# txthpc/amg

Measured on AMD Instinct MI355X. Metric: V-cycle iters/sec + fine-level SpMV GB/s (%HBM peak), 64M-row 7pt Poisson, higher is better.
Workload: dtype f64

## Files before the change

### amg_amd/_native.py

```python
from __future__ import annotations

import ctypes as C
import os
from pathlib import Path

import numpy as np

ROOT = Path(__file__).resolve().parent.parent
LIB_PATH = Path(os.environ["SSS_AMG_LIB"]) if os.environ.get("SSS_AMG_LIB") else ROOT / "amg_amd" / "lib" / "libsss_amg.so"
BIN_PATH = ROOT / "amg_amd" / "bin" / "amg"

_dbl_p = C.POINTER(C.c_double)
_int_p = C.POINTER(C.c_int)


class SSS_MAT(C.Structure):
    _fields_ = [("num_rows", C.c_int), ("num_cols", C.c_int), ("num_nnzs", C.c_int),
                ("row_ptr", _int_p), ("col_idx", _int_p), ("val", _dbl_p)]


class SSS_IMAT(C.Structure):
    _fields_ = [("num_rows", C.c_int), ("num_cols", C.c_int), ("num_nnzs", C.c_int),
                ("row_ptr", _int_p), ("col_idx", _int_p), ("val", _int_p)]


class SSS_VEC(C.Structure):
    _fields_ = [("n", C.c_int), ("d", _dbl_p)]


class SSS_IVEC(C.Structure):
    _fields_ = [("n", C.c_int), ("d", _int_p)]


class SSS_RTN(C.Structure):
    _fields_ = [("ares", C.c_double), ("rres", C.c_double), ("nits", C.c_int)]


class SSS_AMG_PARS(C.Structure):
    _fields_ = [("cycle_type", C.c_int), ("tol", C.c_double), ("ctol", C.c_double), ("max_it", C.c_int),
                ("cs_type", C.c_int), ("max_levels", C.c_int), ("coarse_dof", C.c_int), ("smoother", C.c_int),
                ("relax", C.c_double), ("cf_order", C.c_int), ("pre_iter", C.c_int), ("post_iter", C.c_int),
                ("poly_deg", C.c_int), ("interp_type", C.c_int), ("strong_threshold", C.c_double),
                ("max_row_sum", C.c_double), ("trunc_threshold", C.c_double)]


class SSS_AMG_COMP(C.Structure):
    _fields_ = [("A", SSS_MAT), ("R", SSS_MAT), ("P", SSS_MAT), ("b", SSS_VEC), ("x", SSS_VEC),
                ("cfmark", SSS_IVEC), ("wp", SSS_VEC)]


class SSS_AMG(C.Structure):
    _fields_ = [("num_levels", C.c_int), ("cg", C.POINTER(SSS_AMG_COMP)), ("pars", SSS_AMG_PARS),
                ("rtn", SSS_RTN)]


class SSS_SMTR(C.Structure):
    _fields_ = [("smoother", C.c_int), ("A", C.POINTER(SSS_MAT)), ("b", C.POINTER(SSS_VEC)),
                ("x", C.POINTER(SSS_VEC)), ("relax", C.c_double), ("nsweeps", C.c_int), ("istart", C.c_int),
                ("iend", C.c_int), ("istep", C.c_int), ("ndeg", C.c_int), ("cf_order", C.c_int),
                ("ordering", _int_p)]


class SSS_KRYLOV(C.Structure):
    _fields_ = [("tol", C.c_double), ("A", C.POINTER(SSS_MAT)), ("b", C.POINTER(SSS_VEC)),
                ("u", C.POINTER(SSS_VEC)), ("restart", C.c_int), ("matrix", C.c_int), ("stop_type", C.c_int)]


class SSS_HIP_OPTS(C.Structure):
    _fields_ = [("device", C.c_int), ("smoother", C.c_int), ("coarse", C.c_int), ("row_cap", C.c_int),
                ("use_graph", C.c_int), ("verbose", C.c_int),
                ("inner", C.c_int), ("inner_from", C.c_int), ("relabel", C.c_int),
                ("sorted_tiles", C.c_int), ("sum_order", C.c_int), ("inner_long", C.c_int), ("formats", C.c_int)]

FORMATS = {"auto": -1, "full": 0, "lean": 1}


class SSS_HIP_LEVEL_INFO(C.Structure):
    _fields_ = [("rows", C.c_int), ("nnz", C.c_int), ("nnz_p", C.c_int), ("dag_f", C.c_int),
                ("dag_c", C.c_int), ("smoother_kind", C.c_int), ("gs_engine_f", C.c_int), ("gs_engine_c", C.c_int),
                ("gs_stall", C.c_int), ("a_format", C.c_int), ("a_stream_bytes", C.c_longlong),
                ("inner", C.c_int), ("r_format", C.c_int), ("p_format", C.c_int), ("pad_", C.c_int)]


SMOOTH = {"exact": 0, "hybrid": 1, "jacobi": 2}
COARSE_RS, COARSE_PMIS = 1, 3
COARSE = {"krylov": 0, "direct": 1}
VEC = {"b": 0, "x": 1, "wp": 2}
SPMV = {"mxy": 0, "amxpy": 1, "resid": 2, "acc": 3}

ABI_SYMBOLS = [
    "SSS_amg_solve", "SSS_amg_cycle", "SSS_amg_coarest_solve", "SSS_amg_smoother_pre", "SSS_amg_smoother_post",
    "SSS_blas_mv_amxpy", "SSS_blas_mv_mxy", "SSS_solver_amg", "SSS_get_time", "SSS_free", "SSS_blas_vec_norm2",
    "SSS_print_itinfo", "SSS_exit_on_errcode", "SSS_blas_array_norm2", "SSS_blas_array_dot", "SSS_blas_array_axpy",
    "SSS_blas_array_norminf", "SSS_blas_array_set", "SSS_blas_array_axpby", "SSS_blas_array_ax", "SSS_vec_create",
    "SSS_vec_set_value", "SSS_mat_destroy", "SSS_vec_destroy", "SSS_calloc", "SSS_amg_data_create",
    "SSS_ivec_create", "SSS_mat_struct_create", "SSS_vec_cp", "SSS_iarray_cp", "SSS_blas_array_cp", "SSS_mat_cp",
    "SSS_mat_get_diag", "SSS_ivec_destroy", "SSS_amg_data_destroy", "SSS_imat_trans", "SSS_iarray_set",
    "SSS_imat_destroy", "SSS_mat_trans", "SSS_blas_mat_rap", "SSS_realloc", "SSS_amg_complexity_print",
    "SSS_amg_setup", "SSS_amg_coarsen", "SSS_amg_interp", "SSS_amg_interp_trunc", "interp_DIR", "SSS_mat_read",
    "SSS_amg_pars_init", "SSS_amg_pars_print", "mmio_info", "mmio_data",
    "sss_hip_opts_default", "sss_hip_device_count", "sss_hip_mem_info", "sss_hip_hier_create", "sss_hip_hier_destroy",
    "sss_hip_setup_create", "sss_amg_setup_hooked", "sss_hip_rap", "sss_hip_pmis", "sss_pmis_host",
    "sss_hip_std_pattern", "sss_std_pattern_host", "sss_hip_interp_std",
    "sss_hip_upload_vec", "sss_hip_download_vec", "sss_hip_cycle", "sss_hip_residual_norm", "sss_hip_pcg",
    "sss_hip_fgmres", "sss_hip_host_orth",
    "SSS_amg_save", "SSS_amg_load",
    "sss_hip_coarse_solve", "sss_hip_smooth", "sss_hip_sync", "sss_hip_level_info_get", "sss_hip_num_levels", "sss_hip_tail_from",
    "sss_hip_cycle_launches", "sss_hip_cycle_bytes",
    "sss_hip_spmv_plan_create", "sss_hip_spmv_plan_destroy", "sss_hip_spmv", "sss_hip_host_spmv",
    "sss_hip_host_smooth", "sss_hip_host_coarse_solve", "sss_hip_host_cache_clear", "sss_hip_time_level0_spmv", "sss_hip_time_iterations",
    "sss_hip_time_level0_spmv_csr", "sss_hip_time_levels", "sss_hip_dist_time_tail_levels",
    "sss_gen_stencil",
    "sss_hip_rccl_unique_id", "sss_hip_comm_rccl", "sss_hip_comm_host", "sss_hip_comm_timing", "sss_hip_comm_destroy",
    "sss_hip_dist_create", "sss_hip_dist_destroy", "sss_hip_dist_info", "sss_hip_dist_level_flags",
    "sss_hip_dist_upload_vec",
    "sss_hip_dist_download_vec", "sss_hip_dist_cycle", "sss_hip_dist_residual_norm", "sss_hip_dist_sync",
    "sss_hip_dist_time_level0_spmv", "sss_hip_dist_time_levels", "sss_hip_dist_halo_stats",
    "sss_part_plan_create", "sss_part_plan_destroy", "sss_part_save", "sss_part_plan_load",
    "sss_hip_dist_create_from_files", "sss_hip_dist_level_size", "sss_part_plan_nagg", "sss_part_plan_level",
    "sss_part_plan_matrix", "sss_part_plan_ids", "sss_part_plan_halo",
]

_ip, _dp = C.POINTER(C.c_int), C.POINTER(C.c_double)
EXCHANGE_FN = C.CFUNCTYPE(C.c_int, C.c_void_p, C.c_int, _ip, _ip, _dp, C.c_int, _ip, _ip, _dp)
ALLREDUCE_FN = C.CFUNCTYPE(C.c_int, C.c_void_p, _dp, C.c_int)
ALLGATHERV_FN = C.CFUNCTYPE(C.c_int, C.c_void_p, _dp, C.c_int, _dp, _ip, _ip)


A_FORMATS = {0: "CSR (12 B/entry)", 1: "column-sorted tiles (12 B/entry)", 2: "dictionary tiles (4 B/entry)",
             3: "value-dictionary sorted tiles (5 B/entry)"}


def a_format_name(code: int) -> str:
    if code & 64:
        return "dictionary ELL (1 B/entry, padded rows)"
    if code & 128:
        return "column ELL (4 B/entry, padded rows)"
    return A_FORMATS.get(code & 3, A_FORMATS[0])


class SSS_HIP_HOST_TRANSPORT(C.Structure):
    _fields_ = [("ctx", C.c_void_p), ("exchange", EXCHANGE_FN), ("allreduce_sum", ALLREDUCE_FN),
                ("allgatherv", ALLGATHERV_FN)]

_lib = None


def _declare(lib):
    P = C.POINTER
    sig = {
        "SSS_amg_pars_init": (None, [P(SSS_AMG_PARS)]),
        "SSS_amg_pars_print": (None, [P(SSS_AMG_PARS)]),
        "SSS_amg_setup": (None, [P(SSS_AMG), P(SSS_MAT), P(SSS_AMG_PARS)]),
        "SSS_amg_data_destroy": (None, [P(SSS_AMG)]),
        "SSS_amg_solve": (SSS_RTN, [P(SSS_AMG), P(SSS_VEC), P(SSS_VEC)]),
        "SSS_print_itinfo": (None, [C.c_int, C.c_int, C.c_double, C.c_double, C.c_double]),
        "SSS_amg_cycle": (None, [P(SSS_AMG)]),
        "SSS_solver_amg": (SSS_RTN, [P(SSS_MAT), P(SSS_VEC), P(SSS_VEC), P(SSS_AMG_PARS)]),
        "SSS_mat_read": (None, [C.c_char_p, P(SSS_MAT)]),
        "SSS_mat_destroy": (None, [P(SSS_MAT)]),
        "SSS_mat_trans": (SSS_MAT, [P(SSS_MAT)]),
        "SSS_blas_mat_rap": (SSS_MAT, [P(SSS_MAT), P(SSS_MAT), P(SSS_MAT)]),
        "SSS_amg_coarsen": (C.c_int, [P(SSS_MAT), P(SSS_IVEC), P(SSS_MAT), P(SSS_IMAT), P(SSS_AMG_PARS)]),
        "SSS_amg_interp": (None, [P(SSS_MAT), P(SSS_IVEC), P(SSS_MAT), P(SSS_IMAT), P(SSS_AMG_PARS)]),
        "SSS_ivec_create": (SSS_IVEC, [C.c_int]),
        "SSS_blas_mv_amxpy": (None, [C.c_double, P(SSS_MAT), P(SSS_VEC), P(SSS_VEC)]),
        "SSS_blas_mv_mxy": (None, [P(SSS_MAT), P(SSS_VEC), P(SSS_VEC)]),
        "mmio_info": (C.c_int, [_int_p, _int_p, _int_p, _int_p, C.c_char_p]),
        "mmio_data": (C.c_int, [_int_p, _int_p, _dbl_p, C.c_char_p]),
        "sss_gen_stencil": (C.c_int, [C.c_int] * 6 + [P(SSS_MAT)]),
        "sss_hip_opts_default": (None, [P(SSS_HIP_OPTS)]),
        "sss_hip_device_count": (C.c_int, []),
        "sss_hip_mem_info": (C.c_int, [P(C.c_size_t), P(C.c_size_t)]),
        "sss_hip_hier_create": (C.c_void_p, [P(SSS_AMG), P(SSS_HIP_OPTS)]),
        "sss_hip_setup_create": (C.c_void_p, [P(SSS_AMG), P(SSS_MAT), P(SSS_AMG_PARS), P(SSS_HIP_OPTS),
                                              P(C.c_double)]),
        "sss_hip_hier_destroy": (None, [C.c_void_p]),
        "sss_hip_rap": (C.c_int, [P(SSS_MAT), P(SSS_MAT), P(SSS_MAT), P(SSS_MAT)]),
        "sss_hip_pmis": (C.c_int, [P(SSS_IMAT), _int_p, _int_p, _int_p]),
        "sss_pmis_host": (C.c_int, [P(SSS_IMAT), _int_p, _int_p, _int_p]),
        "sss_hip_std_pattern": (C.c_int, [P(SSS_IMAT), _int_p, C.c_int, P(SSS_MAT)]),
        "sss_std_pattern_host": (C.c_int, [P(SSS_IMAT), _int_p, C.c_int, P(SSS_MAT)]),
        "sss_hip_interp_std": (C.c_int, [P(SSS_MAT), P(SSS_IMAT), _int_p, P(SSS_MAT), C.c_double]),
        "SSS_mat_struct_create": (SSS_MAT, [C.c_int, C.c_int, C.c_int]),
        "sss_hip_upload_vec": (C.c_int, [C.c_void_p, C.c_int, C.c_int, _dbl_p, C.c_int]),
        "sss_hip_download_vec": (C.c_int, [C.c_void_p, C.c_int, C.c_int, _dbl_p, C.c_int]),
        "sss_hip_cycle": (C.c_int, [C.c_void_p]),
        "sss_hip_residual_norm": (C.c_int, [C.c_void_p, _dbl_p]),
        "sss_hip_pcg": (C.c_int, [C.c_void_p, C.c_double, C.c_int, P(C.c_int), _dbl_p, _dbl_p, C.c_int]),
        "sss_hip_fgmres": (C.c_int, [C.c_void_p, C.c_double, C.c_int, C.c_int, P(C.c_int), _dbl_p, _dbl_p, C.c_int]),
        "sss_hip_host_orth": (C.c_int, [C.c_int, C.c_int, _dbl_p, _dbl_p, _dbl_p, _dbl_p]),
        "SSS_amg_save": (C.c_int, [P(SSS_AMG), C.c_char_p]),
        "SSS_amg_load": (C.c_int, [P(SSS_AMG), C.c_char_p]),
        "sss_hip_coarse_solve": (C.c_int, [C.c_void_p]),
        "sss_hip_smooth": (C.c_int, [C.c_void_p, C.c_int, C.c_int]),
        "sss_hip_sync": (C.c_int, [C.c_void_p]),
        "sss_hip_level_info_get": (C.c_int, [C.c_void_p, C.c_int, P(SSS_HIP_LEVEL_INFO)]),
        "sss_hip_num_levels": (C.c_int, [C.c_void_p]),
        "sss_hip_tail_from": (C.c_int, [C.c_void_p]),
        "sss_hip_cycle_launches": (C.c_int, [C.c_void_p]),
        "sss_hip_cycle_bytes": (C.c_int, [C.c_void_p, C.POINTER(C.c_double), C.c_int]),
        "sss_hip_host_spmv": (C.c_int, [C.c_int, C.c_double, P(SSS_MAT), _dbl_p, _dbl_p, _dbl_p, C.c_int]),
        "sss_hip_host_smooth": (C.c_int, [P(SSS_SMTR), C.c_int]),
        "sss_hip_host_coarse_solve": (C.c_int, [P(SSS_MAT), P(SSS_VEC), P(SSS_VEC), C.c_double, C.c_int,
                                                C.c_int]),
        "sss_hip_time_level0_spmv": (C.c_int, [C.c_void_p, C.c_int, _dbl_p]),
        "sss_hip_time_level0_spmv_csr": (C.c_int, [C.c_void_p, C.c_int, _dbl_p]),
        "sss_hip_time_levels": (C.c_int, [C.c_void_p, C.c_int, _dbl_p, C.c_int]),
        "sss_hip_dist_time_tail_levels": (C.c_int, [C.c_void_p, C.c_int, _dbl_p, C.c_int]),
        "sss_hip_time_iterations": (C.c_int, [C.c_void_p, C.c_int, _dbl_p, _dbl_p]),
        "sss_hip_rccl_unique_id": (C.c_int, [C.c_char_p]),
        "sss_hip_comm_rccl": (C.c_void_p, [C.c_int, C.c_int, C.c_char_p, C.c_int]),
        "sss_hip_comm_host": (C.c_void_p, [C.c_int, C.c_int, P(SSS_HIP_HOST_TRANSPORT)]),
        "sss_hip_comm_timing": (C.c_void_p, [C.c_int, C.c_int]),
        "sss_hip_comm_destroy": (None, [C.c_void_p]),
        "sss_hip_dist_create": (C.c_void_p, [P(SSS_AMG), P(SSS_HIP_OPTS), C.c_void_p, C.c_int]),
        "sss_hip_dist_destroy": (None, [C.c_void_p]),
        "sss_hip_dist_info": (C.c_int, [C.c_void_p, _int_p, _int_p, _int_p, _int_p]),
        "sss_hip_dist_level_size": (C.c_int, [C.c_void_p, C.c_int, _int_p, _int_p, P(C.c_longlong)]),
        "sss_hip_dist_level_flags": (C.c_int, [C.c_void_p, C.c_int]),
        "sss_hip_dist_upload_vec": (C.c_int, [C.c_void_p, C.c_int, _dbl_p, C.c_int]),
        "sss_hip_dist_download_vec": (C.c_int, [C.c_void_p, C.c_int, _dbl_p, C.c_int]),
        "sss_hip_dist_cycle": (C.c_int, [C.c_void_p]),
        "sss_hip_dist_residual_norm": (C.c_int, [C.c_void_p, _dbl_p]),
        "sss_hip_dist_sync": (C.c_int, [C.c_void_p]),
        "sss_hip_dist_time_level0_spmv": (C.c_int, [C.c_void_p, C.c_int, _dbl_p]),
        "sss_hip_dist_time_levels": (C.c_int, [C.c_void_p, C.c_int, _dbl_p, _dbl_p, C.c_int]),
        "sss_hip_dist_halo_stats": (C.c_int, [C.c_void_p, P(C.c_longlong), P(C.c_longlong), C.c_int, C.c_int,
                                              _int_p, _int_p, _int_p]),
        "sss_part_plan_create": (C.c_void_p, [P(SSS_AMG), C.c_int, C.c_int, C.c_int]),
        "sss_part_save": (C.c_int, [P(SSS_AMG), C.c_int, C.c_int, C.c_char_p]),
        "sss_part_plan_load": (C.c_void_p, [C.c_char_p]),
        "sss_hip_dist_create_from_files": (C.c_void_p, [C.c_char_p, P(SSS_HIP_OPTS), C.c_void_p]),
        "sss_part_plan_destroy": (None, [C.c_void_p]),
        "sss_part_plan_nagg": (C.c_int, [C.c_void_p]),
        "sss_part_plan_level": (C.c_int, [C.c_void_p, C.c_int, _int_p, _int_p, _int_p, _int_p]),
        "sss_part_plan_matrix": (C.c_int, [C.c_void_p, C.c_int, C.c_int, P(SSS_MAT)]),
        "sss_part_plan_ids": (C.c_int, [C.c_void_p, C.c_int, P(_int_p), P(_int_p)]),
        "sss_part_plan_halo": (C.c_int, [C.c_void_p, C.c_int, _int_p, P(_int_p), P(_int_p), P(_int_p), _int_p,
                                         P(_int_p), P(_int_p)]),
    }
    for name, (res, args) in sig.items():
        fn = getattr(lib, name)
        fn.restype = res
        fn.argtypes = args
    return lib


def lib():
    global _lib
    if _lib is None:
        if not LIB_PATH.exists():
            raise RuntimeError(f"{LIB_PATH} is missing: run `make` (or __graft_entry__.build())")
        _lib = _declare(C.CDLL(str(LIB_PATH)))
    return _lib


def dptr(a: np.ndarray):
    assert a.dtype == np.float64 and a.flags["C_CONTIGUOUS"]
    return a.ctypes.data_as(_dbl_p)


def iptr(a: np.ndarray):
    assert a.dtype == np.int32 and a.flags["C_CONTIGUOUS"]
    return a.ctypes.data_as(_int_p)


def csr_arrays(M: SSS_MAT, copy: bool = True):
    n, nnz = M.num_rows, M.num_nnzs
    rp = np.ctypeslib.as_array(M.row_ptr, shape=(n + 1,))
    ci = np.ctypeslib.as_array(M.col_idx, shape=(nnz,)) if nnz else np.zeros(0, np.int32)
    v = np.ctypeslib.as_array(M.val, shape=(nnz,)) if nnz else np.zeros(0, np.float64)
    return (rp.copy(), ci.copy(), v.copy()) if copy else (rp, ci, v)


class NumpyCSR:

    def __init__(self, rp, ci, v, ncols=None):
        self.rp = np.ascontiguousarray(rp, dtype=np.int32)
        self.ci = np.ascontiguousarray(ci, dtype=np.int32)
        self.v = np.ascontiguousarray(v, dtype=np.float64)
        n = len(self.rp) - 1
        self.mat = SSS_MAT(n, n if ncols is None else ncols, len(self.v), iptr(self.rp), iptr(self.ci),
                           dptr(self.v))


def default_pars() -> SSS_AMG_PARS:
    p = SSS_AMG_PARS()
    lib().SSS_amg_pars_init(C.byref(p))
    return p


def pmis(rp, ci, device: bool = False):
    rp = np.ascontiguousarray(rp, dtype=np.int32)
    ci = np.ascontiguousarray(ci, dtype=np.int32)
    n = len(rp) - 1
    S = SSS_IMAT(n, n, len(ci), iptr(rp), iptr(ci) if len(ci) else None, None)
    mark = np.full(max(n, 1), -7, np.int32)
    nc, rounds = C.c_int(-1), C.c_int(-1)
    fn = lib().sss_hip_pmis if device else lib().sss_pmis_host
    rc = fn(C.byref(S), iptr(mark), C.byref(nc), C.byref(rounds))
    if rc != 0:
        err = RuntimeError(f"PMIS split failed ({rc})")
        err.rc, err.mark = rc, mark[:n]
        raise err
    return mark[:n], nc.value, rounds.value


def _imat(rp, ci):
    rp = np.ascontiguousarray(rp, dtype=np.int32)
    ci = np.ascontiguousarray(ci, dtype=np.int32)
    n = len(rp) - 1
    return SSS_IMAT(n, n, len(ci), iptr(rp), iptr(ci) if len(ci) else None, None), (rp, ci)


def std_pattern(rp, ci, mark, device: bool = False):
    S, keep = _imat(rp, ci)
    mark = np.ascontiguousarray(mark, dtype=np.int32)
    P = SSS_MAT()
    fn = lib().sss_hip_std_pattern if device else lib().sss_std_pattern_host
    rc = fn(C.byref(S), iptr(mark), int((mark == 1).sum()), C.byref(P))
    if rc != 0:
        err = RuntimeError(f"standard pattern failed ({rc})")
        err.rc = rc
        raise err
    prp, pci, _ = csr_arrays(P)
    lib().SSS_mat_destroy(C.byref(P))
    return prp, pci


def interp_std(A_csr, S_csr, mark, P_pattern, trunc: float, device: bool = False):
    Am = NumpyCSR(*A_csr)
    S, keep = _imat(*S_csr)
    mark = np.ascontiguousarray(mark, dtype=np.int32)
    prp = np.ascontiguousarray(P_pattern[0], dtype=np.int32)
    pci = np.ascontiguousarray(P_pattern[1], dtype=np.int32)
    n = len(prp) - 1
    P = lib().SSS_mat_struct_create(n, int((mark == 1).sum()), len(pci))
    C.memmove(P.row_ptr, prp.ctypes.data, prp.nbytes)
    if len(pci):
        C.memmove(P.col_idx, pci.ctypes.data, pci.nbytes)
    try:
        if device:
            rc = lib().sss_hip_interp_std(C.byref(Am.mat), C.byref(S), iptr(mark), C.byref(P), trunc)
            if rc != 0:
                err = RuntimeError(f"standard interpolation failed ({rc})")
                err.rc = rc
                raise err
        else:
            pars = default_pars()
            pars.interp_type, pars.trunc_threshold = 2, trunc
            verts = SSS_IVEC(len(mark), iptr(mark))
            lib().SSS_amg_interp(C.byref(Am.mat), C.byref(verts), C.byref(P), C.byref(S), C.byref(pars))
        return (*csr_arrays(P), P.num_cols)
    finally:
        lib().SSS_mat_destroy(C.byref(P))


def generate(kind: int, n: int, nz: int | None = None, z0: int = 0, z1: int | None = None) -> SSS_MAT:
    nz = n if nz is None else nz
    z1 = nz if z1 is None else z1
    A = SSS_MAT()
    rc = lib().sss_gen_stencil(kind, n, n, nz, z0, z1, C.byref(A))
    if rc != 0:
        raise RuntimeError(f"sss_gen_stencil failed ({rc})")
    return A


def read_mtx(path: str | os.PathLike) -> SSS_MAT:
    A = SSS_MAT()
    lib().SSS_mat_read(str(path).encode(), C.byref(A))
    return A


class Hierarchy:

    def __init__(self, A: SSS_MAT | None, pars: SSS_AMG_PARS | None = None):
        self.pars = pars if pars is not None else default_pars()
        self.mg = SSS_AMG()
        if A is not None:
            lib().SSS_amg_setup(C.byref(self.mg), C.byref(A), C.byref(self.pars))

    def save(self, path) -> None:
        rc = lib().SSS_amg_save(C.byref(self.mg), str(path).encode())
        if rc != 0:
            raise OSError(f"SSS_amg_save({path}) failed ({rc})")

    @classmethod
    def load(cls, path) -> "Hierarchy":
        H = cls(None)
        rc = lib().SSS_amg_load(C.byref(H.mg), str(path).encode())
        if rc != 0:
            raise OSError(f"SSS_amg_load({path}) failed ({rc})")
        H.pars = H.mg.pars
        return H

# ... 425 lines not shown
```

### amg_amd/csrc/sss_hier.hip

```cpp
#include "sss_engine.hpp"
#include "sss_tail.hpp"

#include <atomic>
#include <condition_variable>
#include <mutex>
#include <thread>

#include <chrono>

#include <cmath>

#include <algorithm>
#include <cstdlib>
#include <cstring>
#include <string>
#include <thread>
#include <vector>

using namespace sss;

struct sss_hip_hier {
    int nl = 0;
    SSS_AMG_PARS pars{};
    sss_hip_opts opts{};
// ... 1420 lines not shown
    SSS_HIP(hipEventElapsedTime(&ms, h->ev0, h->ev1));
    *avg_ms = (double)ms / reps;
    return 0;
}

extern "C" int sss_hip_time_iterations(sss_hip_hier *h, int reps, double *avg_ms, double *absres)
{
    SSS_HIP(hipStreamSynchronize(h->stream));
    SSS_HIP(hipEventRecord(h->ev0, h->stream));
    for (int r = 0; r < reps; ++r) {
        int rc = sss_hip_cycle(h);
        if (!rc) rc = sss_hip_residual_norm(h, absres);
        if (rc) return rc;
    }
    SSS_HIP(hipEventRecord(h->ev1, h->stream));
    SSS_HIP(hipEventSynchronize(h->ev1));
    float ms = 0.f;
    SSS_HIP(hipEventElapsedTime(&ms, h->ev0, h->ev1));
    *avg_ms = (double)ms / reps;
    return 0;
}

extern char **environ;

namespace {
struct HostCSR {
    DevCSR d;
    ~HostCSR() { devcsr_free(d); }
};
struct HostSmooth {
    std::mutex run;
    DevCSR d;
    SmootherPlan sp;
    ~HostSmooth()
    {
        smoother_free(sp);
        devcsr_free(d);
    }
};
struct HostCoarse {
    std::mutex run;
    DevCSR d;
    CoarseDirect cd;
    bool direct = false;
    CoarseKrylov *k = nullptr;
    ~HostCoarse()
    {
        if (direct) coarse_direct_free(cd);
        coarse_krylov_destroy(k);
        devcsr_free(d);
    }
};

inline unsigned long long mix64(unsigned long long h, unsigned long long w)
{
    h ^= w * 0x9E3779B97F4A7C15ull;
    h = (h << 31) | (h >> 33);
    return h * 0xC2B2AE3D27D4EB4Full;
}
unsigned long long hash_bytes(const void *p, size_t n, unsigned long long seed)
{
    const unsigned char *b = static_cast<const unsigned char *>(p);
    constexpr size_t kChunk = (size_t)1 << 20;
    const int nc = (int)((n + kChunk - 1) / kChunk);
    std::vector<unsigned long long> part((size_t)std::max(nc, 1), 0);
    parallel_chunks(nc, 1, [&](int c0, int c1) {
        for (int c = c0; c < c1; ++c) {
            const size_t lo = (size_t)c * kChunk, hi = std::min(n, lo + kChunk);
            unsigned long long h = 0x2545F4914F6CDD1Dull ^ (unsigned long long)c;
            size_t i = lo;
            for (; i + 8 <= hi; i += 8) {
                unsigned long long w;
                std::memcpy(&w, b + i, 8);
                h = mix64(h, w);
            }
            for (; i < hi; ++i) h = mix64(h, b[i]);
            part[(size_t)c] = h;
        }
    });
    unsigned long long h = mix64(seed, n);
    for (auto v : part) h = mix64(h, v);
    return h;
}
unsigned long long matrix_key(const SSS_MAT &A, unsigned long long use)
{
    int dev = 0;
    (void)hipGetDevice(&dev);
    unsigned long long h = mix64(mix64(use, (unsigned long long)dev), (unsigned long long)A.num_rows);
    for (char **e = environ; e && *e; ++e)
        if (std::strncmp(*e, "SSS_HIP_", 8) == 0) h = hash_bytes(*e, std::strlen(*e), h);
    h = mix64(h, (unsigned long long)A.num_cols);
    h = mix64(h, (unsigned long long)A.num_nnzs);
    h = hash_bytes(A.row_ptr, sizeof(int) * ((size_t)A.num_rows + 1), h);
    h = hash_bytes(A.col_idx, sizeof(int) * (size_t)A.num_nnzs, h);
    return hash_bytes(A.val, sizeof(double) * (size_t)A.num_nnzs, h);
}

struct PreparedCache {
    struct Entry {
        unsigned long long key;
        std::shared_ptr<void> obj;
        unsigned long long tick;
    };
    std::mutex mu;
    std::vector<Entry> e;
    unsigned long long tick = 0;
    static constexpr size_t kMax = 4;
    template <class T, class Build>
    std::shared_ptr<T> get(unsigned long long key, Build build, bool cache = true)
    {
        if (!cache) return build();
        {
            std::lock_guard<std::mutex> lk(mu);
            for (auto &x : e)
                if (x.key == key) {
                    x.tick = ++tick;
                    return std::static_pointer_cast<T>(x.obj);
                }
        }
        std::shared_ptr<T> obj = build();
        if (!obj) return obj;
        std::lock_guard<std::mutex> lk(mu);
        if (e.size() >= kMax) {
            auto old = std::min_element(e.begin(), e.end(), [](const Entry &a, const Entry &b) { return a.tick < b.tick; });
            e.erase(old);
        }
        e.push_back({key, obj, ++tick});
        return obj;
    }
    void clear()
    {
        std::lock_guard<std::mutex> lk(mu);
        e.clear();
    }
};
bool cacheable(const SSS_MAT &A)
{
    const char *e = getenv("SSS_HIP_HOST_CACHE_MB");
    const double mb = (e && *e) ? atof(e) : 1024.0;
    return 12.0 * (double)A.num_nnzs + 4.0 * (double)A.num_rows <= mb * 1048576.0;
}
PreparedCache &prepared()
{
    static PreparedCache *c = new PreparedCache();
    return *c;
}
}

extern "C" void sss_hip_host_cache_clear(void) { prepared().clear(); }

extern "C" int sss_hip_host_spmv(int op, double alpha, const SSS_MAT *A, const double *x, const double *b,
                                 double *y, int cap)
{
    if (sss_hip_device_count() <= 0) return ERROR_MISC;
    sss_hip_opts o;
    sss_hip_opts_default(&o);
    int enc = level_encoding(o) & (kEncSortedTiles | kEncDict);
    if (A->num_rows != A->num_cols) enc = restriction_encoding(o) & (kEncSortedTiles | kEncEll);
    auto M = prepared().get<HostCSR>(matrix_key(*A, 0x5350ull ^ ((unsigned long long)enc << 8)), [&] {
        auto m = std::make_shared<HostCSR>();
        return devcsr_upload(m->d, *A, -1, enc) ? nullptr : m;
    }, cacheable(*A));
    if (!M) return ERROR_MISC;
    const size_t ny = (size_t)A->num_rows, nx = (size_t)A->num_cols;
    double *dx = dev_alloc<double>(nx), *dy = dev_alloc<double>(ny), *db = dev_alloc<double>(ny);
    int rc = 0;
    if (!dx || !dy || !db) rc = ERROR_ALLOC_MEM;
    if (!rc && hipMemcpy(dx, x, sizeof(double) * nx, hipMemcpyHostToDevice) != hipSuccess) rc = ERROR_MISC;
    if (!rc && hipMemcpy(dy, y, sizeof(double) * ny, hipMemcpyHostToDevice) != hipSuccess) rc = ERROR_MISC;
    if (!rc && b && hipMemcpy(db, b, sizeof(double) * ny, hipMemcpyHostToDevice) != hipSuccess) rc = ERROR_MISC;
    if (!rc) rc = launch_spmv(M->d, op, alpha, dx, db, dy, cap, nullptr, nullptr);
    if (!rc && hipMemcpy(y, dy, sizeof(double) * ny, hipMemcpyDeviceToHost) != hipSuccess) rc = ERROR_MISC;
    dev_free(dx);
    dev_free(dy);
    dev_free(db);
    return rc;
}

extern "C" int sss_hip_host_smooth(const SSS_SMTR *s, int post)
{
    if (sss_hip_device_count() <= 0) return ERROR_MISC;
    const int n = s->A->num_rows;
    const int use_cf = s->cf_order && s->ordering;
    const bool natural = !use_cf && s->smoother == SSS_SM_GS;
    const int i1 = post ? s->iend : s->istart, in = post ? s->istart : s->iend, step = s->istep;
    if (natural && step != 1 && step != -1) {
        fprintf(stderr, "### ERROR: natural-order Gauss-Seidel on the GPU needs istep = +1 or -1 (got %d)\n", step);
        return ERROR_INPUT_PAR;
    }
    const bool desc = step < 0;
    const int lo = desc ? in : i1, hi = (desc ? i1 : in) + 1;
    if (natural && (lo < 0 || hi > n)) return ERROR_INPUT_PAR;
    if (natural && lo >= hi) return 0;
    const int kind = s->smoother == SSS_SM_JACOBI ? SSS_HIP_SMOOTH_JACOBI : SSS_HIP_SMOOTH_EXACT;
    unsigned long long use = mix64(0x534Dull, natural ? 1 : 0);
    use = mix64(use, (unsigned long long)kind);
    if (natural) use = mix64(mix64(use, (unsigned long long)lo), (unsigned long long)hi);
    if (use_cf) use = hash_bytes(s->ordering, sizeof(int) * (size_t)n, use);
    auto M = prepared().get<HostSmooth>(matrix_key(*s->A, use), [&] {
        auto m = std::make_shared<HostSmooth>();
        if (devcsr_upload(m->d, *s->A)) return std::shared_ptr<HostSmooth>();
        if (natural ? smoother_build_natural(m->sp, *s->A, lo, hi)
                    : smoother_build(m->sp, *s->A, use_cf ? s->ordering : nullptr, kind))
            return std::shared_ptr<HostSmooth>();
        return m;
    }, cacheable(*s->A));
    if (!M) return ERROR_MISC;
    std::lock_guard<std::mutex> run_lock(M->run);
    double *dx = dev_alloc<double>((size_t)n), *db = dev_alloc<double>((size_t)n);
    int rc = (!dx || !db) ? ERROR_ALLOC_MEM : 0;
    if (!rc && hipMemcpy(dx, s->x->d, sizeof(double) * n, hipMemcpyHostToDevice) != hipSuccess) rc = ERROR_MISC;
    if (!rc && hipMemcpy(db, s->b->d, sizeof(double) * n, hipMemcpyHostToDevice) != hipSuccess) rc = ERROR_MISC;
    bool x_zero = !natural;
    for (int i = 0; x_zero && i < n; ++i) {
        unsigned long long u;
        memcpy(&u, s->x->d + i, sizeof u);
        x_zero = u == 0ull;
    }
    if (!rc) rc = smoother_run(M->sp, M->d, db, dx, s->nsweeps, nullptr, nullptr, nullptr, nullptr, x_zero, natural && desc);
    if (!rc && hipMemcpy(s->x->d, dx, sizeof(double) * n, hipMemcpyDeviceToHost) != hipSuccess) rc = ERROR_MISC;
    bool stalled = false;
    for (auto &ps : M->sp.pass) {
        unsigned e = 0;
        if (gs_persist_error(ps, &e)) rc = rc ? rc : ERROR_MISC;
        if (e) {
            (void)hipMemset(ps.gp.err, 0, sizeof(unsigned));
            stalled = true;
        }
    }
    unsigned ez = 0;
    if (gs_fused_error(M->sp.fz, &ez, true)) rc = rc ? rc : ERROR_MISC;
    if (ez) stalled = true;
    if (stalled && !rc) rc = stall_error("SSS_amg_smoother_pre/post");
    dev_free(dx);
    dev_free(db);
    return rc;
}

extern "C" int sss_hip_host_coarse_solve(SSS_MAT *A, SSS_VEC *b, SSS_VEC *x, double ctol, int coarse_mode,
                                         int row_cap)
{
    if (sss_hip_device_count() <= 0) return ERROR_MISC;
    const int n = A->num_rows;
    const bool direct = coarse_mode == SSS_HIP_COARSE_DIRECT && n <= 20000;
    auto M = prepared().get<HostCoarse>(
        matrix_key(*A, mix64(mix64(0x4353ull, direct ? 1 : 0), (unsigned long long)row_cap)), [&] {
            auto m = std::make_shared<HostCoarse>();
            if (devcsr_upload(m->d, *A)) return std::shared_ptr<HostCoarse>();
            if (direct) {
                if (coarse_direct_build(m->cd, *A, nullptr)) return std::shared_ptr<HostCoarse>();
                m->direct = true;
            } else {
                m->k = coarse_krylov_create(m->d, row_cap, nullptr);
                if (!m->k) return std::shared_ptr<HostCoarse>();
            }
            return m;
        }, cacheable(*A));
    if (!M) return ERROR_MISC;
    std::lock_guard<std::mutex> run_lock(M->run);
    double *dx = dev_alloc<double>((size_t)n), *db = dev_alloc<double>((size_t)n);
    int rc = (!dx || !db) ? ERROR_ALLOC_MEM : 0;
    if (!rc && hipMemcpy(dx, x->d, sizeof(double) * n, hipMemcpyHostToDevice) != hipSuccess) rc = ERROR_MISC;
    if (!rc && hipMemcpy(db, b->d, sizeof(double) * n, hipMemcpyHostToDevice) != hipSuccess) rc = ERROR_MISC;
    if (!rc) {
        if (direct) {
            rc = coarse_direct_apply(M->cd, db, dx, nullptr);
            if (!rc && hipDeviceSynchronize() != hipSuccess) rc = ERROR_MISC;
        } else {
            rc = coarse_krylov_solve(M->k, M->d, db, dx, ctol, nullptr);
        }
    }
    if (!rc && hipMemcpy(x->d, dx, sizeof(double) * n, hipMemcpyDeviceToHost) != hipSuccess) rc = ERROR_MISC;
    dev_free(dx);
    dev_free(db);
    return rc;
}
```

### amg_amd/csrc/sss_spmv_dev.hpp

```cpp
#pragma once

#include "sss_engine.hpp"

namespace sss {

__device__ __forceinline__ int xcd_bid() { return blockIdx.x; }

struct SpmvSmem {
    alignas(16) double v[kTileEntries];
    double red[kBlock / 64];
    double d[kBlock];
};

struct DictSmem {
    int dd[256];
    double vd[256];
    unsigned char rowof[kTileEntries];
};
struct DevDict {
    const unsigned *code = nullptr;
    const int4 *pd = nullptr;
    const int *dd = nullptr;
    const double *vd = nullptr;
    const unsigned *pk = nullptr;
// ... 680 lines not shown
        const double acc = long_row_chunks(
            k0, k1, b[i], [=, &sm](int base, int m) { stage_products(sm.v, base, base + m, ci, v, x); },
            [&sm](int, int m, double acc) { return threadIdx.x == 0 ? chain_sub(acc, sm.v, 0, m) : acc; });
        if (threadIdx.x == 0) epi(r0, i, acc);
    }
}
constexpr int kWaveStage = 256;
constexpr int kWaveRowMin = 600;
constexpr int kFreeRowMin = 300;

__device__ __forceinline__ void wave_sync()
{
    __builtin_amdgcn_fence(__ATOMIC_RELEASE, "wavefront");
    __builtin_amdgcn_wave_barrier();
    __builtin_amdgcn_fence(__ATOMIC_ACQUIRE, "wavefront");
}

template <bool SUB, class Prod>
__device__ __forceinline__ double wave_row_chain(int k0, int k1, const int *__restrict__ ci,
                                                 const double *__restrict__ v, Prod prod, double init,
                                                 double *strip)
{
    constexpr int U = kWaveStage / 64;
    const int lane = threadIdx.x & 63;
    double acc = init;
    for (int base = k0; base < k1; base += kWaveStage) {
        const int m = min(kWaveStage, k1 - base);
        int c[U];
        double a[U];
#pragma unroll
        for (int u = 0; u < U; ++u) {
            const int q = lane + 64 * u, qc = q < m ? q : m - 1;
            const int cv = ci[base + qc];
            const double av = v[base + qc];
            c[u] = cv;
            a[u] = q < m ? av : 0.0;
        }
        double pv[U];
#pragma unroll
        for (int u = 0; u < U; ++u) pv[u] = prod(c[u], a[u]);
#pragma unroll
        for (int u = 0; u < U; ++u) {
            const int q = lane + 64 * u;
            if (q < m) strip[q] = pv[u];
        }
        wave_sync();
        if (lane == 0) acc = chain_pipe16<SUB>(acc, strip, 0, m);
        wave_sync();
    }
    return acc;
}

template <class Prod>
__device__ __forceinline__ double wave_row_sum(int k0, int k1, const int *__restrict__ ci,
                                               const double *__restrict__ v, Prod prod)
{
    constexpr int U = 4;
    const int lane = threadIdx.x & 63;
    double s0 = 0.0, s1 = 0.0;
    for (int k = k0 + lane; k < k1; k += 64 * U) {
        int c[U];
        double a[U];
#pragma unroll
        for (int u = 0; u < U; ++u) {
            const int kk = k + 64 * u, kc = kk < k1 ? kk : k1 - 1;
            const int cv = ci[kc];
            const double av = v[kc];
            c[u] = cv;
            a[u] = kk < k1 ? av : 0.0;
        }
        double pv[U];
#pragma unroll
        for (int u = 0; u < U; ++u) pv[u] = prod(c[u], a[u]);
#pragma unroll
        for (int u = 0; u < U; ++u) {
            const double p = k + 64 * u < k1 ? pv[u] : 0.0;
            if (u & 1) s1 += p;
            else s0 += p;
        }
    }
    double s = s0 + s1;
#pragma unroll
    for (int off = 32; off > 0; off >>= 1) s += __shfl_xor(s, off, 64);
    return s;
}



template <int G, int S, class Fetch>
__device__ __forceinline__ void merged_sums(int k0, int k1, const unsigned *__restrict__ mk,
                                            const double *__restrict__ mv, Fetch fetch, double (&s0)[G],
                                            double (&s1)[G])
{
    constexpr int U = 8;
    const int lane = threadIdx.x & 63;
#pragma unroll
    for (int u = 0; u < G; ++u) s0[u] = 0.0, s1[u] = 0.0;
    for (int k = k0 + lane; k < k1 && S == 2; k += 64 * U) {
        unsigned q[U];
        double a[U];
#pragma unroll
        for (int t = 0; t < U; ++t) {
            const int kk = k + 64 * t;
            q[t] = kk < k1 ? mk[kk] : 0u;
            a[t] = kk < k1 ? mv[kk] : 0.0;
        }
#pragma unroll
        for (int t = 0; t < U; ++t) {
            if (k + 64 * t >= k1) break;
            const double p = a[t] * fetch((int)(q[t] >> kMergeShift));
            const unsigned key = q[t] & ((1u << kMergeShift) - 1);
#pragma unroll
            for (int u = 0; u < G; ++u) {
                s0[u] += key == (unsigned)u ? p : 0.0;
                s1[u] += key == (unsigned)(8 + u) ? p : 0.0;
            }
        }
    }
    for (int k = k0 + lane; k < k1 && S == 1; k += 64 * U) {
        unsigned q[U];
        double a[U], xv[U];
#pragma unroll
        for (int t = 0; t < U; ++t) {
            const int kk = k + 64 * t, kc = kk < k1 ? kk : k1 - 1;
            q[t] = mk[kc];
            a[t] = mv[kc];
        }
#pragma unroll
        for (int t = 0; t < U; ++t) xv[t] = k + 64 * t < k1 ? fetch((int)(q[t] >> kMergeShift)) : 0.0;
#pragma unroll
        for (int t = 0; t < U; ++t) {
            const bool live = k + 64 * t < k1;
            const double p = live ? a[t] * xv[t] : 0.0;
            const unsigned key = live ? q[t] & ((1u << kMergeShift) - 1) : 0u;
#pragma unroll
            for (int u = 0; u < G; ++u) {
                s0[u] += key == (unsigned)u ? p : 0.0;
                if (S == 2) s1[u] += key == (unsigned)(8 + u) ? p : 0.0;
            }
        }
    }
#pragma unroll
    for (int u = 0; u < G; ++u)
#pragma unroll
        for (int off = 32; off > 0; off >>= 1) {
            s0[u] += __shfl_xor(s0[u], off, 64);
            if (S == 2) s1[u] += __shfl_xor(s1[u], off, 64);
        }
}

constexpr int kMergeAccDoubles = 64;
template <int S>
constexpr int kMergeLdsChunks = S == 2 ? 6 : 8;
template <int G, int S, int C, class Fetch>
__device__ __forceinline__ void merged_batch_lds(const unsigned *__restrict__ pk, const double *__restrict__ pv,
                                                 int last_n, Fetch fetch, double *mine)
{
    const int lane = threadIdx.x & 63;
    const int ll = min(lane, last_n - 1);
    unsigned q[C];
    double a[C], xv[C];
#pragma unroll
    for (int t = 0; t < C; ++t) {
        const int o = 64 * t + (t == C - 1 ? ll : lane);
        q[t] = pk[o];
        a[t] = pv[o];
    }
#pragma unroll
    for (int t = 0; t < C; ++t) xv[t] = fetch((int)(q[t] >> kMergeShift));
#pragma unroll
    for (int t = 0; t < C; ++t) {
        const unsigned key = q[t] & ((1u << kMergeShift) - 1);
        const unsigned slot = S == 2 ? (key >> 3) * G + (key & (G - 1)) : key & (G - 1);
        double p = a[t] * xv[t];
        if (t == C - 1) p = lane < last_n ? p : 0.0;
        atomicAdd(&mine[slot * kMergeAccDoubles], p);
    }
}
template <int G, int S, int C, class Fetch>
__device__ __forceinline__ void merged_batch_dispatch(int nch, const unsigned *__restrict__ pk,
                                                      const double *__restrict__ pv, int last_n, Fetch fetch,
                                                      double *mine)
{
    if constexpr (C == 1) {
        merged_batch_lds<G, S, 1>(pk, pv, last_n, fetch, mine);
    } else {
        if (nch == C) merged_batch_lds<G, S, C>(pk, pv, last_n, fetch, mine);
        else merged_batch_dispatch<G, S, C - 1>(nch, pk, pv, last_n, fetch, mine);
    }
}
template <int G, int S, class Fetch>
__device__ __forceinline__ void merged_sums_lds(int k0, int k1, const unsigned *__restrict__ mk,
                                                const double *__restrict__ mv, Fetch fetch, double *acc,
                                                double (&s0)[G], double (&s1)[G])
{
    constexpr int U = kMergeLdsChunks<S>;
    const int lane = threadIdx.x & 63;
    double *mine = acc + lane;
#pragma unroll
    for (int a = 0; a < S * G; ++a) mine[a * kMergeAccDoubles] = 0.0;
    k1 = __builtin_amdgcn_readfirstlane(k1);
    for (int kb = __builtin_amdgcn_readfirstlane(k0); kb < k1; kb += 64 * U) {
        const int rem = min(k1 - kb, 64 * U), nch = (rem + 63) >> 6, last_n = rem - 64 * (nch - 1);
        const unsigned *pk = mk + kb;
        const double *pv = mv + kb;
        merged_batch_dispatch<G, S, U>(nch, pk, pv, last_n, fetch, mine);
    }
#pragma unroll
    for (int u = 0; u < G; ++u) {
        s0[u] = mine[u * kMergeAccDoubles];
        s1[u] = S == 2 ? mine[(G + u) * kMergeAccDoubles] : 0.0;
    }
#pragma unroll
    for (int u = 0; u < G; ++u)
#pragma unroll
        for (int off = 32; off > 0; off >>= 1) {
            s0[u] += __shfl_xor(s0[u], off, 64);
            if (S == 2) s1[u] += __shfl_xor(s1[u], off, 64);
        }
}

template <int G, int S, bool LDSACC, class Fetch>
__device__ __forceinline__ bool merged_block(const int *__restrict__ gp, int ng, int W, const unsigned *__restrict__ mk,
                                             const double *__restrict__ mv, Fetch fetch, double *red, double *acc,
                                             int &g_out, int &u_out, double &t0, double &t1)
{
    const int w = threadIdx.x >> 6, lane = threadIdx.x & 63, gpb = 4 / W;
    const int g = xcd_bid() * gpb + w / W, part = w % W;
    double s0[G], s1[G];
    if (g < ng) {
        const int k0 = gp[g], k1 = gp[g + 1], len = k1 - k0, per = (len + W - 1) / W;
        if constexpr (LDSACC)
            merged_sums_lds<G, S>(k0 + min(len, part * per), k0 + min(len, (part + 1) * per), mk, mv, fetch,
                                  acc + w * (S * G * kMergeAccDoubles), s0, s1);
        else
            merged_sums<G, S>(k0 + min(len, part * per), k0 + min(len, (part + 1) * per), mk, mv, fetch, s0, s1);
    } else {
#pragma unroll
        for (int u = 0; u < G; ++u) s0[u] = 0.0, s1[u] = 0.0;
    }
    if (lane == 0)
#pragma unroll
        for (int u = 0; u < G; ++u) {
            red[(w * 2) * G + u] = s0[u];
            if (S == 2) red[(w * 2 + 1) * G + u] = s1[u];
        }
    __syncthreads();
    const int t = threadIdx.x;
    if (t >= gpb * G) return false;
    const int gi = t / G, u = t % G, gg = xcd_bid() * gpb + gi;
    if (gg >= ng) return false;
    double a0 = red[((gi * W) * 2) * G + u], a1 = S == 2 ? red[((gi * W) * 2 + 1) * G + u] : 0.0;
    for (int v = 1; v < W; ++v) {
        a0 += red[((gi * W + v) * 2) * G + u];
        if (S == 2) a1 += red[((gi * W + v) * 2 + 1) * G + u];
    }
    g_out = gg, u_out = u, t0 = a0, t1 = a1;
    return true;
}

}
```

### include/sss_hip.h

```cpp
#ifndef SSS_HIP_H
#define SSS_HIP_H

#include "sss_amg.h"

#ifdef __cplusplus
extern "C" {
#endif

enum {
    SSS_HIP_SMOOTH_EXACT = 0,
    SSS_HIP_SMOOTH_HYBRID = 1,
    SSS_HIP_SMOOTH_JACOBI = 2
};
enum {
    SSS_HIP_COARSE_KRYLOV = 0,
    SSS_HIP_COARSE_DIRECT = 1
};
enum { SSS_HIP_VEC_B = 0, SSS_HIP_VEC_X = 1, SSS_HIP_VEC_WP = 2 };

typedef struct sss_hip_opts {
    int device;
    int smoother;
    int coarse;
    int row_cap;
    int use_graph;
    int verbose;
    int inner;
    int inner_from;
    int relabel;
    int sorted_tiles;
    int sum_order;
    int inner_long;
    int formats;
} sss_hip_opts;

#define SSS_HIP_LONG_ROW_MIN 300
void sss_hip_opts_default(sss_hip_opts *o);

int sss_hip_device_count(void);
int sss_hip_mem_info(size_t *free_bytes, size_t *total_bytes);

typedef struct sss_hip_hier sss_hip_hier;

sss_hip_hier *sss_hip_hier_create(const SSS_AMG *mg, const sss_hip_opts *o);
void sss_hip_hier_destroy(sss_hip_hier *h);

sss_hip_hier *sss_hip_setup_create(SSS_AMG *mg, SSS_MAT *A, SSS_AMG_PARS *pars, const sss_hip_opts *o,
                                   double *times);

int sss_hip_rap(const SSS_MAT *R, const SSS_MAT *A, const SSS_MAT *P, SSS_MAT *C);

#define SSS_SETUP_GPU_PMIS_MIN_DEFAULT 10000000
int sss_hip_pmis(const SSS_IMAT *S, int *mark, int *ncoarse, int *rounds);
int sss_pmis_host(const SSS_IMAT *S, int *mark, int *ncoarse, int *rounds);

#define SSS_SETUP_GPU_INTERP_MIN_DEFAULT 10000000
int sss_hip_std_pattern(const SSS_IMAT *S, const int *mark, int ncoarse, SSS_MAT *P);
int sss_hip_interp_std(const SSS_MAT *A, const SSS_IMAT *S, const int *mark, SSS_MAT *P, double trunc_threshold);
int sss_std_pattern_host(const SSS_IMAT *S, const int *mark, int ncoarse, SSS_MAT *P);

typedef void (*sss_setup_hook)(void *ctx, const SSS_AMG *mg, int done, int final);
void sss_amg_setup_hooked(SSS_AMG *mg, SSS_MAT *A, SSS_AMG_PARS *pars, sss_setup_hook hook, void *ctx);

int sss_hip_upload_vec(sss_hip_hier *h, int level, int which, const double *src, int n);
int sss_hip_download_vec(sss_hip_hier *h, int level, int which, double *dst, int n);

int sss_hip_cycle(sss_hip_hier *h);
int sss_hip_residual_norm(sss_hip_hier *h, double *absres);
int SSS_amg_save(const SSS_AMG *mg, const char *path);
int SSS_amg_load(SSS_AMG *mg, const char *path);

int sss_hip_pcg(sss_hip_hier *h, double tol, int maxit, int *iters, double *relres, double *hist, int hist_cap);
int sss_hip_fgmres(sss_hip_hier *h, double tol, int restart, int maxit, int *iters, double *relres, double *hist,
                   int hist_cap);
int sss_hip_coarse_solve(sss_hip_hier *h);
int sss_hip_smooth(sss_hip_hier *h, int level, int post);
int sss_hip_sync(sss_hip_hier *h);

typedef struct sss_hip_level_info {
    int rows, nnz, nnz_p, dag_f, dag_c, smoother_kind;
    int gs_engine_f, gs_engine_c, gs_stall, a_format;
    long long a_stream_bytes;
    int inner;
    int r_format, p_format;
    int pad_;
} sss_hip_level_info;
int sss_hip_level_info_get(sss_hip_hier *h, int level, sss_hip_level_info *out);
int sss_hip_num_levels(sss_hip_hier *h);
int sss_hip_tail_from(sss_hip_hier *h);
int sss_hip_cycle_launches(sss_hip_hier *h);
int sss_hip_cycle_bytes(sss_hip_hier *h, double *out, int nslots);

enum {
    SSS_HIP_SPMV_MXY = 0,
    SSS_HIP_SPMV_AMXPY = 1,
    SSS_HIP_SPMV_RESID = 2,
    SSS_HIP_SPMV_ACC = 3
};
typedef struct sss_hip_spmv_plan sss_hip_spmv_plan;
sss_hip_spmv_plan *sss_hip_spmv_plan_create(int n, int nnz, const int *d_rp, const int *h_rp);
void sss_hip_spmv_plan_destroy(sss_hip_spmv_plan *p);
int sss_hip_spmv(const sss_hip_spmv_plan *p, int op, double alpha, const int *d_rp, const int *d_ci,
                 const double *d_v, const double *d_x, const double *d_b, double *d_y, int cap,
                 void *stream);

int sss_hip_host_spmv(int op, double alpha, const SSS_MAT *A, const double *x, const double *b,
                      double *y, int cap);
int sss_hip_host_smooth(const SSS_SMTR *s, int post);
int sss_hip_host_orth(int n, int k, const double *V, double *w, double *hcol, double *norm);
void sss_hip_host_cache_clear(void);
int sss_hip_host_coarse_solve(SSS_MAT *A, SSS_VEC *b, SSS_VEC *x, double ctol, int coarse_mode,
                              int row_cap);

int sss_hip_time_level0_spmv(sss_hip_hier *h, int reps, double *avg_ms);
int sss_hip_time_levels(sss_hip_hier *h, int reps, double *level_ms, int nslots);
int sss_hip_time_level0_spmv_csr(sss_hip_hier *h, int reps, double *avg_ms);
int sss_hip_time_iterations(sss_hip_hier *h, int reps, double *avg_ms, double *absres);

typedef struct sss_hip_comm sss_hip_comm;
typedef struct sss_hip_dist sss_hip_dist;
typedef struct sss_hip_host_transport {
    void *ctx;
    int (*exchange)(void *ctx, int nsend, const int *sdst, const int *scount, const double *sbuf, int nrecv,
                    const int *rsrc, const int *rcount, double *rbuf);
    int (*allreduce_sum)(void *ctx, double *v, int n);
    int (*allgatherv)(void *ctx, const double *mine, int count, double *all, const int *counts, const int *displs);
} sss_hip_host_transport;

#define SSS_HIP_RCCL_ID_BYTES 128
int sss_hip_rccl_unique_id(unsigned char *id);
sss_hip_comm *sss_hip_comm_rccl(int nranks, int rank, const unsigned char *id, int device);
sss_hip_comm *sss_hip_comm_host(int nranks, int rank, const sss_hip_host_transport *t);
sss_hip_comm *sss_hip_comm_timing(int nranks, int rank);
void sss_hip_comm_destroy(sss_hip_comm *c);

sss_hip_dist *sss_hip_dist_create(const SSS_AMG *mg, const sss_hip_opts *o, sss_hip_comm *c, int agg_rows);
sss_hip_dist *sss_hip_dist_create_from_files(const char *prefix, const sss_hip_opts *o, sss_hip_comm *c);
void sss_hip_dist_destroy(sss_hip_dist *d);
int sss_hip_dist_info(sss_hip_dist *d, int *lo, int *hi, int *nagg, int *nghost0);
int sss_hip_dist_level_size(sss_hip_dist *d, int l, int *m, int *g, long long *nnz);
int sss_hip_dist_level_flags(sss_hip_dist *d, int l);
int sss_hip_dist_upload_vec(sss_hip_dist *d, int which, const double *own, int n);
int sss_hip_dist_download_vec(sss_hip_dist *d, int which, double *own, int n);
int sss_hip_dist_cycle(sss_hip_dist *d);
int sss_hip_dist_residual_norm(sss_hip_dist *d, double *absres);
int sss_hip_dist_sync(sss_hip_dist *d);
int sss_hip_dist_time_level0_spmv(sss_hip_dist *d, int reps, double *avg_ms);
int sss_hip_dist_time_levels(sss_hip_dist *d, int reps, double *cycle_ms, double *level_ms, int nslots);
int sss_hip_dist_time_tail_levels(sss_hip_dist *d, int reps, double *level_ms, int nslots);
int sss_hip_dist_halo_stats(sss_hip_dist *d, long long *calls, long long *doubles, int nslots, int reset,
                            int *nc_own, int *nc_all, int *tail_levels);

typedef struct sss_part_plan sss_part_plan;
sss_part_plan *sss_part_plan_create(const SSS_AMG *mg, int nranks, int rank, int agg_rows);
int sss_part_save(const SSS_AMG *mg, int nranks, int agg_rows, const char *prefix);
sss_part_plan *sss_part_plan_load(const char *path);
void sss_part_plan_destroy(sss_part_plan *p);
int sss_part_plan_nagg(const sss_part_plan *p);
int sss_part_plan_level(const sss_part_plan *p, int l, int *lo, int *hi, int *m, int *g);
int sss_part_plan_matrix(const sss_part_plan *p, int l, int which, SSS_MAT *out);
int sss_part_plan_ids(const sss_part_plan *p, int l, const int **perm, const int **ghosts);
int sss_part_plan_halo(const sss_part_plan *p, int l, int *nsend, const int **sdst, const int **scount,
                       const int **sidx, int *nrecv, const int **rsrc, const int **rcount);

int sss_gen_stencil(int kind, int nx, int ny, int nz, int z0, int z1, SSS_MAT *A);

#ifdef __cplusplus
}
#endif
#endif
```

Measured before the change: 53.72.

## Restructure merged-row LDS accumulators with key-indexed layout and tree reduction

Changes the LDS accumulator layout in the merged SpMV path so the packed key bits index slots directly, which removes the per-element slot arithmetic. The per-lane shuffle reductions are replaced by a transposed tree reduction across the wave that writes results straight into the reduction buffer. Wave-partition arithmetic now uses shifts and readfirstlane. It also adds a host SpMV entry point with a selectable summation order and lets the Python loader tolerate missing symbols. The trade-off is a different floating-point summation order and more complex LDS indexing.

```diff
diff --git a/amg_amd/_native.py b/amg_amd/_native.py
--- a/amg_amd/_native.py
+++ b/amg_amd/_native.py
@@ -107,7 +107,7 @@
     "SSS_amg_save", "SSS_amg_load",
     "sss_hip_coarse_solve", "sss_hip_smooth", "sss_hip_sync", "sss_hip_level_info_get", "sss_hip_num_levels", "sss_hip_tail_from",
     "sss_hip_cycle_launches", "sss_hip_cycle_bytes",
-    "sss_hip_spmv_plan_create", "sss_hip_spmv_plan_destroy", "sss_hip_spmv", "sss_hip_host_spmv",
+    "sss_hip_spmv_plan_create", "sss_hip_spmv_plan_destroy", "sss_hip_spmv", "sss_hip_host_spmv", "sss_hip_host_spmv_order",
     "sss_hip_host_smooth", "sss_hip_host_coarse_solve", "sss_hip_host_cache_clear", "sss_hip_time_level0_spmv", "sss_hip_time_iterations",
     "sss_hip_time_level0_spmv_csr", "sss_hip_time_levels", "sss_hip_dist_time_tail_levels",
     "sss_gen_stencil",
@@ -201,6 +201,7 @@
         "sss_hip_cycle_launches": (C.c_int, [C.c_void_p]),
         "sss_hip_cycle_bytes": (C.c_int, [C.c_void_p, C.POINTER(C.c_double), C.c_int]),
         "sss_hip_host_spmv": (C.c_int, [C.c_int, C.c_double, P(SSS_MAT), _dbl_p, _dbl_p, _dbl_p, C.c_int]),
+        "sss_hip_host_spmv_order": (C.c_int, [C.c_int, C.c_double, P(SSS_MAT), _dbl_p, _dbl_p, _dbl_p, C.c_int, C.c_int]),
         "sss_hip_host_smooth": (C.c_int, [P(SSS_SMTR), C.c_int]),
         "sss_hip_host_coarse_solve": (C.c_int, [P(SSS_MAT), P(SSS_VEC), P(SSS_VEC), C.c_double, C.c_int,
                                                 C.c_int]),
@@ -241,7 +242,12 @@
                                          P(_int_p), P(_int_p)]),
     }
     for name, (res, args) in sig.items():
-        fn = getattr(lib, name)
+        try:
+            fn = getattr(lib, name)
+        except AttributeError:
+            if os.environ.get("SSS_AMG_LIB"):
+                continue
+            raise
         fn.restype = res
         fn.argtypes = args
     return lib
diff --git a/amg_amd/csrc/sss_hier.hip b/amg_amd/csrc/sss_hier.hip
--- a/amg_amd/csrc/sss_hier.hip
+++ b/amg_amd/csrc/sss_hier.hip
@@ -1596,11 +1596,19 @@
 extern "C" int sss_hip_host_spmv(int op, double alpha, const SSS_MAT *A, const double *x, const double *b,
                                  double *y, int cap)
 {
+    return sss_hip_host_spmv_order(op, alpha, A, x, b, y, cap, 0);
+}
+
+extern "C" int sss_hip_host_spmv_order(int op, double alpha, const SSS_MAT *A, const double *x, const double *b,
+                                       double *y, int cap, int sum_order)
+{
     if (sss_hip_device_count() <= 0) return ERROR_MISC;
     sss_hip_opts o;
     sss_hip_opts_default(&o);
-    int enc = level_encoding(o) & (kEncSortedTiles | kEncDict);
-    if (A->num_rows != A->num_cols) enc = restriction_encoding(o) & (kEncSortedTiles | kEncEll);
+    o.sum_order = sum_order == 1 ? 1 : 0;
+    const int order = o.sum_order == 1 ? kEncFreeOrder : 0;
+    int enc = level_encoding(o) & (kEncSortedTiles | kEncDict | order);
+    if (A->num_rows != A->num_cols) enc = restriction_encoding(o) & (kEncSortedTiles | kEncEll | order);
     auto M = prepared().get<HostCSR>(matrix_key(*A, 0x5350ull ^ ((unsigned long long)enc << 8)), [&] {
         auto m = std::make_shared<HostCSR>();
         return devcsr_upload(m->d, *A, -1, enc) ? nullptr : m;
diff --git a/amg_amd/csrc/sss_spmv_dev.hpp b/amg_amd/csrc/sss_spmv_dev.hpp
--- a/amg_amd/csrc/sss_spmv_dev.hpp
+++ b/amg_amd/csrc/sss_spmv_dev.hpp
@@ -856,6 +856,19 @@
 constexpr int kMergeAccDoubles = 64;
 template <int S>
 constexpr int kMergeLdsChunks = S == 2 ? 6 : 8;
+template <int G, int S>
+constexpr unsigned kMergeKeyMask = S == 2 ? (8u | (unsigned)(G - 1)) : (unsigned)(G - 1);
+template <int G, int S>
+__device__ __forceinline__ constexpr int merged_acc_key(int a)
+{
+    return S == 2 ? (a / G) << 3 | (a % G) : a;
+}
+template <int G, int S>
+__device__ __forceinline__ int merged_acc_base(int w)
+{
+    if (S == 2 && G == 4) return ((w >> 1) * 16 + (w & 1) * 4) * kMergeAccDoubles;
+    return w * (S * G * kMergeAccDoubles);
+}
 template <int G, int S, int C, class Fetch>
 __device__ __forceinline__ void merged_batch_lds(const unsigned *__restrict__ pk, const double *__restrict__ pv,
                                                  int last_n, Fetch fetch, double *mine)
@@ -874,11 +887,11 @@
     for (int t = 0; t < C; ++t) xv[t] = fetch((int)(q[t] >> kMergeShift));
 #pragma unroll
     for (int t = 0; t < C; ++t) {
-        const unsigned key = q[t] & ((1u << kMergeShift) - 1);
-        const unsigned slot = S == 2 ? (key >> 3) * G + (key & (G - 1)) : key & (G - 1);
+        static_assert(kMergeKeyMask<G, S> < (1u << kMergeShift), "key bits");
+        const unsigned key = q[t] & kMergeKeyMask<G, S>;
         double p = a[t] * xv[t];
         if (t == C - 1) p = lane < last_n ? p : 0.0;
-        atomicAdd(&mine[slot * kMergeAccDoubles], p);
+        atomicAdd(&mine[key * kMergeAccDoubles], p);
     }
 }
 template <int G, int S, int C, class Fetch>
@@ -893,16 +906,36 @@
         else merged_batch_dispatch<G, S, C - 1>(nch, pk, pv, last_n, fetch, mine);
     }
 }
+template <int G, int S>
+__device__ __forceinline__ void merged_tree_lds(const double *acc, double *out)
+{
+    constexpr int NA = S * G, LP = 64 / NA;
+    static_assert(NA >= 2 && NA <= 32 && LP * NA == 64, "accumulators per wave");
+    const int lane = threadIdx.x & 63, a = lane / LP, i = lane % LP;
+    const double *col = acc + merged_acc_key<G, S>(a) * kMergeAccDoubles + i;
+    wave_sync();
+    double v[NA];
+#pragma unroll
+    for (int m = 0; m < NA; ++m) v[m] = col[LP * m];
+#pragma unroll
+    for (int h = NA / 2; h > 0; h >>= 1)
+#pragma unroll
+        for (int m = 0; m < h; ++m) v[m] += v[m + h];
+    double s = v[0];
+#pragma unroll
+    for (int off = LP / 2; off > 0; off >>= 1) s += __shfl_xor(s, off, 64);
+    if (i == 0) out[a] = s;
+}
 template <int G, int S, class Fetch>
 __device__ __forceinline__ void merged_sums_lds(int k0, int k1, const unsigned *__restrict__ mk,
                                                 const double *__restrict__ mv, Fetch fetch, double *acc,
-                                                double (&s0)[G], double (&s1)[G])
+                                                double *out)
 {
     constexpr int U = kMergeLdsChunks<S>;
     const int lane = threadIdx.x & 63;
     double *mine = acc + lane;
 #pragma unroll
-    for (int a = 0; a < S * G; ++a) mine[a * kMergeAccDoubles] = 0.0;
+    for (int a = 0; a < S * G; ++a) mine[merged_acc_key<G, S>(a) * kMergeAccDoubles] = 0.0;
     k1 = __builtin_amdgcn_readfirstlane(k1);
     for (int kb = __builtin_amdgcn_readfirstlane(k0); kb < k1; kb += 64 * U) {
         const int rem = min(k1 - kb, 64 * U), nch = (rem + 63) >> 6, last_n = rem - 64 * (nch - 1);
@@ -910,18 +943,7 @@
         const double *pv = mv + kb;
         merged_batch_dispatch<G, S, U>(nch, pk, pv, last_n, fetch, mine);
     }
-#pragma unroll
-    for (int u = 0; u < G; ++u) {
-        s0[u] = mine[u * kMergeAccDoubles];
-        s1[u] = S == 2 ? mine[(G + u) * kMergeAccDoubles] : 0.0;
-    }
-#pragma unroll
-    for (int u = 0; u < G; ++u)
-#pragma unroll
-        for (int off = 32; off > 0; off >>= 1) {
-            s0[u] += __shfl_xor(s0[u], off, 64);
-            if (S == 2) s1[u] += __shfl_xor(s1[u], off, 64);
-        }
+    merged_tree_lds<G, S>(acc, out);
 }
 
 template <int G, int S, bool LDSACC, class Fetch>
@@ -929,35 +951,39 @@
                                              const double *__restrict__ mv, Fetch fetch, double *red, double *acc,
                                              int &g_out, int &u_out, double &t0, double &t1)
 {
-    const int w = threadIdx.x >> 6, lane = threadIdx.x & 63, gpb = 4 / W;
-    const int g = xcd_bid() * gpb + w / W, part = w % W;
-    double s0[G], s1[G];
-    if (g < ng) {
-        const int k0 = gp[g], k1 = gp[g + 1], len = k1 - k0, per = (len + W - 1) / W;
-        if constexpr (LDSACC)
-            merged_sums_lds<G, S>(k0 + min(len, part * per), k0 + min(len, (part + 1) * per), mk, mv, fetch,
-                                  acc + w * (S * G * kMergeAccDoubles), s0, s1);
-        else
+    const int w = __builtin_amdgcn_readfirstlane(threadIdx.x >> 6), lane = threadIdx.x & 63;
+    const int wsh = W >= 4 ? 2 : W >= 2 ? 1 : 0, gpb = 4 >> wsh;
+    const int g = xcd_bid() * gpb + (w >> wsh), part = w & ((1 << wsh) - 1);
+    if (LDSACC && g < ng) {
+        const int k0 = gp[g], k1 = gp[g + 1], len = k1 - k0, per = (len + (1 << wsh) - 1) >> wsh;
+        merged_sums_lds<G, S>(k0 + min(len, part * per), k0 + min(len, (part + 1) * per), mk, mv, fetch,
+                              acc + merged_acc_base<G, S>(w), red + (w * 2) * G);
+    } else {
+        double s0[G], s1[G];
+        if (g < ng) {
+            const int k0 = gp[g], k1 = gp[g + 1], len = k1 - k0, per = (len + (1 << wsh) - 1) >> wsh;
             merged_sums<G, S>(k0 + min(len, part * per), k0 + min(len, (part + 1) * per), mk, mv, fetch, s0, s1);
-    } else {
-#pragma unroll
-        for (int u = 0; u < G; ++u) s0[u] = 0.0, s1[u] = 0.0;
-    }
-    if (lane == 0)
-#pragma unroll
-        for (int u = 0; u < G; ++u) {
-            red[(w * 2) * G + u] = s0[u];
-            if (S == 2) red[(w * 2 + 1) * G + u] = s1[u];
-        }
+        } else {
+#pragma unroll
+            for (int u = 0; u < G; ++u) s0[u] = 0.0, s1[u] = 0.0;
+        }
+        if (lane == 0)
+#pragma unroll
+            for (int u = 0; u < G; ++u) {
+                red[(w * 2) * G + u] = s0[u];
+                if (S == 2) red[(w * 2 + 1) * G + u] = s1[u];
+            }
+    }
     __syncthreads();
     const int t = threadIdx.x;
     if (t >= gpb * G) return false;
     const int gi = t / G, u = t % G, gg = xcd_bid() * gpb + gi;
     if (gg >= ng) return false;
-    double a0 = red[((gi * W) * 2) * G + u], a1 = S == 2 ? red[((gi * W) * 2 + 1) * G + u] : 0.0;
-    for (int v = 1; v < W; ++v) {
-        a0 += red[((gi * W + v) * 2) * G + u];
-        if (S == 2) a1 += red[((gi * W + v) * 2 + 1) * G + u];
+    const int w0 = gi << wsh;
+    double a0 = red[(w0 * 2) * G + u], a1 = S == 2 ? red[(w0 * 2 + 1) * G + u] : 0.0;
+    for (int v = 1; v < (1 << wsh); ++v) {
+        a0 += red[((w0 + v) * 2) * G + u];
+        if (S == 2) a1 += red[((w0 + v) * 2 + 1) * G + u];
     }
     g_out = gg, u_out = u, t0 = a0, t1 = a1;
     return true;
diff --git a/include/sss_hip.h b/include/sss_hip.h
--- a/include/sss_hip.h
+++ b/include/sss_hip.h
@@ -106,6 +106,8 @@
 
 int sss_hip_host_spmv(int op, double alpha, const SSS_MAT *A, const double *x, const double *b,
                       double *y, int cap);
+int sss_hip_host_spmv_order(int op, double alpha, const SSS_MAT *A, const double *x, const double *b,
+                            double *y, int cap, int sum_order);
 int sss_hip_host_smooth(const SSS_SMTR *s, int post);
 int sss_hip_host_orth(int n, int k, const double *V, double *w, double *hcol, double *norm);
 void sss_hip_host_cache_clear(void);
```

New measurement: 54.40 (median of 6 runs). 1.3% higher.
